# al-mcintyre/mCaller

Measured on NVIDIA B200. Metric: per-read site calls/sec, higher is better.
Workload: dtype f64

## Files before the change

### mcaller_b200/csrc/common.cuh

```cuda
#pragma once
#include <cuda_runtime.h>
#include <stdint.h>
#include <stdio.h>
#include "../../include/mcaller_b200.h"

void mc_set_error(const char *fmt, ...);

#define MC_CUDA_CHECK(expr)                                                                  \
    do {                                                                                     \
        cudaError_t _e = (expr);                                                             \
        if (_e != cudaSuccess) {                                                             \
            mc_set_error("%s:%d %s -> %s", __FILE__, __LINE__, #expr, cudaGetErrorString(_e)); \
            return MC_ECUDA;                                                                 \
        }                                                                                    \
    } while (0)

#define MC_LAUNCH_CHECK() MC_CUDA_CHECK(cudaGetLastError())

#define MC_REQUIRE(cond, msg)                       \
    do {                                            \
        if (!(cond)) {                              \
            mc_set_error("%s: %s", __func__, msg);  \
            return MC_EINVAL;                       \
        }                                           \
    } while (0)

__device__ __forceinline__ uint32_t mc_kmer_bits(const uint32_t *__restrict__ bm, int64_t g, int k) {
    int64_t w = g >> 5;
    int b = (int)(g & 31);
    uint32_t lo = __ldg(bm + w), hi = __ldg(bm + w + 1);
    uint32_t v = __funnelshift_r(lo, hi, b);
    return v & ((1u << k) - 1u);
}

template <int THREADS>
__device__ __forceinline__ int mc_block_exscan(int v, int *s_warp , int &total) {
    const int lane = threadIdx.x & 31, wid = threadIdx.x >> 5;
    int inc = v;
#pragma unroll
    for (int d = 1; d < 32; d <<= 1) {
        int t = __shfl_up_sync(0xffffffffu, inc, d);
        if (lane >= d) inc += t;
    }
    if (lane == 31) s_warp[wid] = inc;
    __syncthreads();
    if (wid == 0) {
        int x = (lane < THREADS / 32) ? s_warp[lane] : 0;
        int xi = x;
#pragma unroll
        for (int d = 1; d < 32; d <<= 1) {
            int t = __shfl_up_sync(0xffffffffu, xi, d);
            if (lane >= d) xi += t;
        }
        if (lane < THREADS / 32) s_warp[lane] = xi - x;
        if (lane == 31) s_warp[THREADS / 32] = xi;
    }
    __syncthreads();
    total = s_warp[THREADS / 32];
    int res = s_warp[wid] + inc - v;
    __syncthreads();
    return res;
}

int mc_exscan_u32(const uint32_t *d_in, uint32_t *d_out, int64_t n_cap, const uint64_t *d_n ,
                  uint64_t *d_total , void *d_ws, cudaStream_t st);
int64_t mc_exscan_ws_bytes(int64_t n);

__device__ __forceinline__ int64_t mc_dev_count(const unsigned long long *d_n, int64_t cap) {
    const unsigned long long v = *d_n;
    return v < (unsigned long long)cap ? (int64_t)v : cap;
}

__device__ __forceinline__ int64_t mc_rec_line(const mc_record &r) { return ((int64_t)r.line_hi << 32) | (int64_t)r.line_lo; }

struct mc_read_key {
    unsigned long long hash;
    uint32_t check;
    uint32_t len;
};
__device__ __forceinline__ mc_read_key mc_read_key_of(const uint8_t *p, int64_t max_len) {
    unsigned long long h = 14695981039346656037ull, h2 = 0x84222325cbf29ce4ull;
    int64_t len = 0;
    for (; len < max_len; ++len) {
        const unsigned c = __ldg(p + len);
        if (c <= 0x20u || c == ':' || c == '_') break;
        h = (h ^ c) * 1099511628211ull;
        h2 = (h2 ^ c) * 1099511628211ull;
    }
    return {h == 0ull ? 1ull : h, (uint32_t)(h2 >> 32), (uint32_t)len};
}

template <class F>
__device__ __forceinline__ double mc_pairwise_block(F f, int64_t i0, int64_t n) {
    if (n < 8) {
        double res = 0.0;
        for (int64_t i = 0; i < n; ++i) res = __dadd_rn(res, f(i0 + i));
        return res;
    }
    double r[8];
#pragma unroll
    for (int j = 0; j < 8; ++j) r[j] = f(i0 + j);
    int64_t i = 8;
    for (; i < n - (n % 8); i += 8) {
#pragma unroll
        for (int j = 0; j < 8; ++j) r[j] = __dadd_rn(r[j], f(i0 + i + j));
    }
    double res = __dadd_rn(__dadd_rn(__dadd_rn(r[0], r[1]), __dadd_rn(r[2], r[3])), __dadd_rn(__dadd_rn(r[4], r[5]), __dadd_rn(r[6], r[7])));
    for (; i < n; ++i) res = __dadd_rn(res, f(i0 + i));
    return res;
}
template <class F>
__device__ double mc_pairwise_sum(F f, int64_t i0, int64_t n) {
    if (n <= 128) return mc_pairwise_block(f, i0, n);
    constexpr int DEPTH = 40;
    int64_t st_i0[DEPTH], st_n[DEPTH];
    double st_left[DEPTH];
    int st_phase[DEPTH];
    int sp = 0;
    st_i0[0] = i0; st_n[0] = n; st_phase[0] = 0; st_left[0] = 0.0;
    double ret = 0.0;
    for (;;) {
        if (st_phase[sp] == 0) {
            if (st_n[sp] <= 128 || sp + 1 >= DEPTH) {
                ret = mc_pairwise_block(f, st_i0[sp], st_n[sp]);
            } else {
                int64_t n2 = st_n[sp] / 2;
                n2 -= n2 % 8;
                st_phase[sp] = 1;
                st_i0[sp + 1] = st_i0[sp]; st_n[sp + 1] = n2; st_phase[sp + 1] = 0;
                ++sp;
                continue;
            }
        }
        for (;;) {
            if (sp == 0) return ret;
            --sp;
            if (st_phase[sp] == 1) {
                int64_t n2 = st_n[sp] / 2;
                n2 -= n2 % 8;
                st_left[sp] = ret;
                st_phase[sp] = 2;
                st_i0[sp + 1] = st_i0[sp] + n2; st_n[sp + 1] = st_n[sp] - n2; st_phase[sp + 1] = 0;
                ++sp;
                break;
            }
            ret = __dadd_rn(st_left[sp], ret);
        }
    }
}

__device__ __forceinline__ double mc_expit(double x) { return x < 0.0 ? exp(x) / (1.0 + exp(x)) : 1.0 / (1.0 + exp(-x)); }

__device__ __forceinline__ double mc_tanh(double x) {
    double y = -2.0 * fabs(x);
    y = fmax(y, -80.0);
    const double n = rint(y * 1.4426950408889634074);
    double r = fma(n, -6.93147180369123816490e-01, y);
    r = fma(n, -1.90821492927058770002e-10, r);
    double p = 1.6059043836821613e-10;
    p = fma(p, r, 2.0876756987868100e-09);
    p = fma(p, r, 2.5052108385441720e-08);
    p = fma(p, r, 2.7557319223985890e-07);
    p = fma(p, r, 2.7557319223985893e-06);
    p = fma(p, r, 2.4801587301587302e-05);
    p = fma(p, r, 1.9841269841269841e-04);
    p = fma(p, r, 1.3888888888888889e-03);
    p = fma(p, r, 8.3333333333333332e-03);
    p = fma(p, r, 4.1666666666666664e-02);
    p = fma(p, r, 1.6666666666666666e-01);
    p = fma(p, r, 0.5);
    p = fma(p, r, 1.0);
    p = fma(p, r, 1.0);
    const double t = p * __longlong_as_double((long long)(1023 + (int)n) << 52);
    const double d = 1.0 + t, u = 1.0 - t;
    double rc = (double)__frcp_rn((float)d);
    double e = fma(-d, rc, 1.0);
    rc = fma(rc, e, rc);
    e = fma(-d, rc, 1.0);
    rc = fma(rc, e, rc);
    double q = u * rc;
    q = fma(fma(-d, q, u), rc, q);
    return copysign(q, x);
}
```

### mcaller_b200/csrc/parse.cuh

```cuda
#pragma once
#include "common.cuh"

__constant__ double c_pow10[23] = {1e0,  1e1,  1e2,  1e3,  1e4,  1e5,  1e6,  1e7,  1e8,  1e9,  1e10, 1e11,
                                   1e12, 1e13, 1e14, 1e15, 1e16, 1e17, 1e18, 1e19, 1e20, 1e21, 1e22};

struct SmemBytes {
    const uint8_t *p;
    __device__ __forceinline__ int operator[](int i) const { return p[i]; }
};
struct GlobalBytes {
    const uint8_t *p;
    int64_t limit;
    __device__ __forceinline__ int operator[](int64_t i) const { return i < limit ? __ldg(p + i) : 0x0a; }
};

template <class B>
__device__ __forceinline__ bool contig_match(const B &t, int q, const mc_refindex &R, int cid) {
    const int o0 = __ldg(R.d_name_off + cid), L = __ldg(R.d_name_off + cid + 1) - o0;
    for (int j = 0; j < L; ++j)
        if (t[q + j] != __ldg(R.d_names + o0 + j)) return false;
    return t[q + L] <= 0x20;
}
template <class B>
__device__ __forceinline__ int contig_cmp(const B &t, int q, const mc_refindex &R, int cid) {
    const int o0 = __ldg(R.d_name_off + cid), L = __ldg(R.d_name_off + cid + 1) - o0;
    for (int j = 0; j < L; ++j) {
        const int a = t[q + j], b = __ldg(R.d_names + o0 + j);
        if (a <= 0x20) return -1;
        if (a != b) return a - b;
    }
    return t[q + L] <= 0x20 ? 0 : 1;
}
template <class B>
__device__ __forceinline__ int contig_lookup(const B &t, int q, const mc_refindex &R, int hint) {
    if (contig_match(t, q, R, hint)) return hint;
    int lo = 0, hi = R.n_contigs - 1;
    while (lo <= hi) {
        const int mid = (lo + hi) >> 1;
        const int c = contig_cmp(t, q, R, mid);
        if (c == 0) return mid;
        if (c < 0) hi = mid - 1; else lo = mid + 1;
    }
    return -1;
}
template <class B>
__device__ __forceinline__ bool parse_uint(const B &t, int q, int &out) {
    int v = 0, nd = 0, c;
    while ((c = t[q]) >= '0' && c <= '9') { v = v * 10 + (c - '0'); ++nd; ++q; if (nd > 9) return false; }
    if (nd == 0 || c > 0x20) return false;
    out = v;
    return true;
}
template <class B>
__device__ __forceinline__ bool parse_int(const B &t, int q, int &out) {
    bool neg = false;
    if (t[q] == '-') { neg = true; ++q; } else if (t[q] == '+') ++q;
    int v;
    if (!parse_uint(t, q, v)) return false;
    out = neg ? -v : v;
    return true;
}
template <class B>
__device__ __forceinline__ bool parse_decimal(const B &t, int q, double &out) {
    bool neg = false;
    int c = t[q];
    if (c == '-') { neg = true; ++q; } else if (c == '+') ++q;
    unsigned long long m = 0;
    int nd = 0, nfrac = 0;
    while ((c = t[q]) >= '0' && c <= '9') { m = m * 10ull + (unsigned)(c - '0'); ++nd; ++q; if (nd > 18) return false; }
    if (c == '.') {
        ++q;
        while ((c = t[q]) >= '0' && c <= '9') { m = m * 10ull + (unsigned)(c - '0'); ++nd; ++nfrac; ++q; if (nd > 18) return false; }
    }
    if (nd == 0 || c > 0x20 || m > (1ull << 53)) return false;
    const double v = __ddiv_rn((double)m, c_pow10[nfrac]);
    out = neg ? -v : v;
    return true;
}
template <class B>
__device__ __forceinline__ bool is_nnnnnn(const B &t, int q) {
    if (t[q] != 'N') return false;
    return t[q + 1] == 'N' && t[q + 2] == 'N' && t[q + 3] == 'N' && t[q + 4] == 'N' && t[q + 5] == 'N' && t[q + 6] <= 0x20;
}


template <class B>
__device__ __forceinline__ bool tokens_equal(const B &t, int64_t a, int64_t b) {
    for (;;) {
        const int ca = t[a++], cb = t[b++];
        const bool ea = ca <= 0x20, eb = cb <= 0x20;
        if (ea || eb) return ea && eb;
        if (ca != cb) return false;
    }
}

template <class B>
__device__ __forceinline__ void parse_values(const B &t, int f2, int f5, int f6, int f9, int f10, int &event_idx, double &diff,
                                             uint32_t &flags) {
    event_idx = 0;
    if (!parse_int(t, f5, event_idx)) flags |= MC_RF_BADIDX;
    double ev = 0.0, md = 0.0;
    if (!parse_decimal(t, f6, ev) || !parse_decimal(t, f10, md)) { flags |= MC_RF_BADNUM; diff = 0.0; }
    else diff = __ddiv_rn(rint(__dmul_rn(__dsub_rn(ev, md), 1e4)), 1e4);
    if (tokens_equal(t, f2, f9)) flags |= MC_RF_EQ;
}

__device__ __forceinline__ uint32_t gt20_msb(uint32_t w) { return (((w & 0x7f7f7f7fu) + 0x5f5f5f5fu) | w) & 0x80808080u; }
__device__ __forceinline__ uint32_t pack16(uint32_t m0, uint32_t m1, uint32_t m2, uint32_t m3) {
    const uint32_t lo = 0x08040201u, hi = 0x80402010u;
    const uint32_t a = __dp4a(m1, hi, __dp4a(m0, lo, 0u)), b = __dp4a(m3, hi, __dp4a(m2, lo, 0u));
    return (a >> 7) | (b << 1);
}
__device__ __forceinline__ int nth_bit(uint32_t m, int j) {
#pragma unroll
    for (int t = 0; t < 6; ++t)
        if (j > t) m &= m - 1u;
    for (int t = 6; t < j; ++t) m &= m - 1u;
    return __ffs(m) - 1;
}
__device__ __forceinline__ uint32_t conv4(uint32_t h) {
    const uint32_t t = ((h * 2561u) >> 8) & 0x00ff00ffu;
    return (t * 6553601u) >> 16;
}

__device__ __forceinline__ unsigned long long nondigit8(unsigned long long v) {
    const unsigned long long x = v ^ 0x3030303030303030ull;
    return (((x & 0x7f7f7f7f7f7f7f7full) + 0x7676767676767676ull) | v) & 0x8080808080808080ull;
}
__device__ __forceinline__ uint32_t digits_value(unsigned long long v, int n) {
    const unsigned long long x = (v ^ 0x3030303030303030ull) << (64 - 8 * n);
    return conv4((uint32_t)x) * 10000u + conv4((uint32_t)(x >> 32));
}
__device__ __forceinline__ bool fast_uint8(unsigned long long v, int &out) {
    const unsigned long long nd = nondigit8(v);
    if (nd == 0ull) return false;
    const int n = (__ffsll((long long)nd) - 1) >> 3;
    if (n == 0 || ((v >> (8 * n)) & 0xFFull) > 0x20ull) return false;
    out = (int)digits_value(v, n);
    return true;
}
__device__ __forceinline__ bool fast_decimal8(unsigned long long v, uint32_t &mant, int &nfrac) {
    const unsigned long long nd = nondigit8(v);
    if (nd == 0ull) return false;
    const int p1 = (__ffsll((long long)nd) - 1) >> 3;
    if (p1 == 0 || p1 > 6 || ((v >> (8 * p1)) & 0xFFull) != 0x2eull) return false;
    const unsigned long long low = (1ull << (8 * p1)) - 1ull;
    const unsigned long long w = (v & low) | ((v >> 8) & ~low);
    const unsigned long long nd2 = ((nd & low) | ((nd >> 8) & ~low)) & 0x0080808080808080ull;
    if (nd2 == 0ull) return false;
    const int p2 = (__ffsll((long long)nd2) - 1) >> 3;
    if (((w >> (8 * p2)) & 0xFFull) > 0x20ull) return false;
    mant = digits_value(w, p2);
    nfrac = p2 - p1;
    return true;
}
__device__ __forceinline__ int fast_tokens_equal8(unsigned long long a, unsigned long long b) {
    auto ws8 = [](unsigned long long v) {
        return ~((((v & 0x7f7f7f7f7f7f7f7full) + 0x5f5f5f5f5f5f5f5full) | v)) & 0x8080808080808080ull;
    };
    const unsigned long long wa = ws8(a), wb = ws8(b);
    if (wa == 0ull || wb == 0ull) return -1;
    const int la = (__ffsll((long long)wa) - 1) >> 3, lb = (__ffsll((long long)wb) - 1) >> 3;
    if (la != lb) return 0;
    return (((a ^ b) & ((1ull << (8 * la)) - 1ull)) == 0ull) ? 1 : 0;
}

__device__ __forceinline__ unsigned long long load8_unaligned(const uint8_t *p) {
    const uintptr_t a = reinterpret_cast<uintptr_t>(p);
    const unsigned long long *q = reinterpret_cast<const unsigned long long *>(a & ~(uintptr_t)7);
    const int sh = 8 * (int)(a & 7);
    const unsigned long long lo = __ldg(q);
    if (sh == 0) return lo;
    const unsigned long long hi = __ldg(q + 1);
    return (lo >> sh) | (hi << (64 - sh));
}
__device__ __forceinline__ bool bytes_differ(const uint8_t *pa, const uint8_t *pb, int L) {
    const uintptr_t ua = reinterpret_cast<uintptr_t>(pa), ub = reinterpret_cast<uintptr_t>(pb);
    const unsigned long long *qa = reinterpret_cast<const unsigned long long *>(ua & ~(uintptr_t)7);
    const unsigned long long *qb = reinterpret_cast<const unsigned long long *>(ub & ~(uintptr_t)7);
    const int sa = 8 * (int)(ua & 7), sb = 8 * (int)(ub & 7);
    unsigned long long a_lo = __ldg(qa), b_lo = __ldg(qb), diff = 0ull;
#pragma unroll 5
    for (int j = 0; j < L; j += 8) {
        const unsigned long long a_hi = __ldg(++qa), b_hi = __ldg(++qb);
        const unsigned long long va = sa ? ((a_lo >> sa) | (a_hi << (64 - sa))) : a_lo;
        const unsigned long long vb = sb ? ((b_lo >> sb) | (b_hi << (64 - sb))) : b_lo;
        unsigned long long d = va ^ vb;
        if (L - j < 8) d &= (1ull << (8 * (L - j))) - 1ull;
        diff |= d;
        a_lo = a_hi;
        b_lo = b_hi;
    }
    return diff != 0ull;
}

__device__ __forceinline__ void mc_finish_values(const uint8_t *lp, int64_t room, int f2, int f5, int f6, int f9, int f10, int &ev_idx,
                                                 double &diff, uint32_t &fl) {
    uint32_t m_ev = 0u, m_md = 0u;
    int n_ev = 0, n_md = 0;
    const int teq = fast_tokens_equal8(load8_unaligned(lp + f2), load8_unaligned(lp + f9));
    if (f10 + 16 < room && teq >= 0 && fast_uint8(load8_unaligned(lp + f5), ev_idx) &&
        fast_decimal8(load8_unaligned(lp + f6), m_ev, n_ev) && fast_decimal8(load8_unaligned(lp + f10), m_md, n_md)) {
        const double ev = __ddiv_rn((double)m_ev, c_pow10[n_ev]), md = __ddiv_rn((double)m_md, c_pow10[n_md]);
        diff = __ddiv_rn(rint(__dmul_rn(__dsub_rn(ev, md), 1e4)), 1e4);
        if (teq) fl |= MC_RF_EQ;
    } else {
        parse_values(GlobalBytes{lp, room}, f2, f5, f6, f9, f10, ev_idx, diff, fl);
    }
}

__device__ __forceinline__ void mc_finish_record(const uint8_t *__restrict__ text, int64_t limit, mc_record &r) {
    const int64_t line = mc_rec_line(r);
    const int64_t a0 = line & ~15ll;
    const int skip = (int)(line - a0);
    int nf = 0, f2 = 0, f3 = 0, name_end = -1, f5 = 0, f6 = 0, f9 = 0, f10 = 0;
    uint32_t prev_nonws = 0u;
    bool done = false;
    constexpr int MAX_STEPS = 256;
    for (int step = 0; step < MAX_STEPS && !done; ++step) {
        const int64_t g = a0 + 16ll * step;
        if (g >= limit) break;
        const uint4 v = __ldg(reinterpret_cast<const uint4 *>(text + g));
        uint32_t nonws = pack16(gt20_msb(v.x), gt20_msb(v.y), gt20_msb(v.z), gt20_msb(v.w));
        if (step == 0) nonws &= 0xFFFFu << skip;
        const int base = 16 * step - skip;
        uint32_t fs = nonws & ~((nonws << 1) | prev_nonws);
        if (name_end < 0 && nf >= 4) {
            const uint32_t z = ~nonws & 0xFFFFu & ((step == 0) ? (0xFFFFu << skip) : 0xFFFFu);
            const uint32_t zz = z & ~((1u << max(f3 - base, 0)) - 1u);
            if (zz) name_end = base + __ffs(zz) - 1;
        }
        while (fs) {
            const int b = __ffs(fs) - 1;
            fs &= fs - 1u;
            const int pos = base + b;
            switch (nf) {
                case 2: f2 = pos; break;
                case 3: f3 = pos; break;
                case 5: f5 = pos; break;
                case 6: f6 = pos; break;
                case 9: f9 = pos; break;
                case 10: f10 = pos; break;
                default: break;
            }
            ++nf;
            if (nf == 4 && name_end < 0) {
                const uint32_t z = ~nonws & 0xFFFFu & ~((1u << b) - 1u);
                if (z) name_end = base + __ffs(z) - 1;
            }
            if (nf == 11) { done = true; break; }
        }
        prev_nonws = (nonws >> 15) & 1u;
    }
    uint32_t fl = r.flags & ~MC_RF_RAW;
    int ev_idx = 0;
    double diff = 0.0;
    if (nf < 11 || name_end < 0 || f3 > 65535 || name_end - f3 > 65535) fl |= MC_RF_BADNUM | MC_RF_BADIDX;
    else mc_finish_values(text + line, limit - line, f2, f5, f6, f9, f10, ev_idx, diff, fl);
    r.name_off = (uint16_t)f3;
    r.name_len = (uint16_t)(name_end < 0 ? 0 : name_end - f3);
    r.event_idx = ev_idx;
    r.diff = diff;
    r.flags = (uint8_t)fl;
}

__device__ __forceinline__ void mc_finish_record_win(const uint8_t *__restrict__ text, int64_t limit, mc_record &r) {
    const uint32_t *rw = reinterpret_cast<const uint32_t *>(&r);
    const uint32_t W0 = rw[3], W1 = rw[4], W2 = rw[5], W3 = (rw[1] >> 16) | (rw[6] << 16);
    const int c0 = __popc(W0), c1 = c0 + __popc(W1), c2 = c1 + __popc(W2), c3 = c2 + __popc(W3);
    const int64_t line = mc_rec_line(r);
    if ((r.pad & 2u) || c3 < 11 || line + 160 >= limit) {
        r.pad = 0;
        mc_finish_record(text, limit, r);
        return;
    }
    uint32_t m = W0;
    int wi = 0;
    auto next = [&]() {
        while (m == 0u && wi < 3) {
            ++wi;
            m = wi == 1 ? W1 : wi == 2 ? W2 : W3;
        }
        const int q = 32 * wi + __ffs(m) - 1;
        m &= m - 1u;
        return q;
    };
    next();
    next();
    const int f2 = next(), f3 = next(), f4 = next(), f5 = next(), f6 = next();
    next();
    next();
    const int f9 = next(), f10 = next();
    const uint8_t *lp = text + line;
    int name_end;
    {
        const unsigned long long t8 = f4 >= 8 ? load8_unaligned(lp + f4 - 8) : 0ull;
        const uint32_t nh = gt20_msb((uint32_t)(t8 >> 32)), nlw = gt20_msb((uint32_t)t8);
        const int tw = nh ? (__clz(nh) >> 3) : nlw ? 4 + (__clz(nlw) >> 3) : 8;
        name_end = f4 - tw;
        if (tw == 8 || name_end <= f3) {
            name_end = f4 - 1;
            while (name_end > f3 && __ldg(lp + name_end - 1) <= 0x20) --name_end;
        }
    }
    uint32_t fl = r.flags & ~MC_RF_RAW;
    int ev_idx = 0;
    double diff = 0.0;
    mc_finish_values(lp, limit - line, f2, f5, f6, f9, f10, ev_idx, diff, fl);
    r.name_off = (uint16_t)f3;
    r.name_len = (uint16_t)(name_end - f3);
    r.event_idx = ev_idx;
    r.diff = diff;
    r.flags = (uint8_t)fl;
    r.pad = 0;
}
```

### mcaller_b200/csrc/records.cu

```cuda
#include "parse.cuh"

namespace {

constexpr int SCAN_THREADS = 256;
constexpr int SCAN_IPT = 8;
constexpr int SCAN_BLOCK = SCAN_THREADS * SCAN_IPT;

__global__ void __launch_bounds__(SCAN_THREADS) k_scan_reduce(const uint32_t *__restrict__ in, int64_t n_cap,
                                                            const unsigned long long *__restrict__ d_n,
                                                            unsigned long long *__restrict__ block_sums) {
    __shared__ int s_warp[SCAN_THREADS / 32 + 1];
    const int64_t n = d_n ? mc_dev_count(d_n, n_cap) : n_cap;
    const int64_t base = (int64_t)blockIdx.x * SCAN_BLOCK;
    unsigned long long acc = 0ull;
#pragma unroll
    for (int j = 0; j < SCAN_IPT; ++j) {
        const int64_t i = base + (int64_t)j * SCAN_THREADS + threadIdx.x;
        if (i < n) acc += in[i];
    }
    for (int d = 16; d > 0; d >>= 1) acc += __shfl_down_sync(0xffffffffu, acc, d);
    __shared__ unsigned long long s_sum[SCAN_THREADS / 32];
    if ((threadIdx.x & 31) == 0) s_sum[threadIdx.x >> 5] = acc;
    __syncthreads();
    if (threadIdx.x == 0) {
        unsigned long long t = 0ull;
        for (int w = 0; w < SCAN_THREADS / 32; ++w) t += s_sum[w];
        block_sums[blockIdx.x] = t;
    }
    (void)s_warp;
}

__global__ void __launch_bounds__(1024) k_scan_sums(unsigned long long *__restrict__ block_sums, int64_t nb,
                                                   unsigned long long *__restrict__ d_total) {
    __shared__ unsigned long long s_w[33];
    __shared__ unsigned long long s_carry;
    if (threadIdx.x == 0) s_carry = 0ull;
    __syncthreads();
    const int lane = threadIdx.x & 31, wid = threadIdx.x >> 5;
    for (int64_t c0 = 0; c0 < nb; c0 += 1024) {
        const int64_t i = c0 + threadIdx.x;
        const unsigned long long v = (i < nb) ? block_sums[i] : 0ull;
        unsigned long long inc = v;
        for (int d = 1; d < 32; d <<= 1) {
            unsigned long long t = __shfl_up_sync(0xffffffffu, inc, d);
            if (lane >= d) inc += t;
        }
        if (lane == 31) s_w[wid] = inc;
        __syncthreads();
        if (wid == 0) {
            unsigned long long x = s_w[lane], xi = x;
            for (int d = 1; d < 32; d <<= 1) {
                unsigned long long t = __shfl_up_sync(0xffffffffu, xi, d);
                if (lane >= d) xi += t;
            }
            s_w[lane] = xi - x;
            if (lane == 31) s_w[32] = xi;
        }
        __syncthreads();
        const unsigned long long carry = s_carry;
        if (i < nb) block_sums[i] = carry + s_w[wid] + inc - v;
        __syncthreads();
        if (threadIdx.x == 0) s_carry = carry + s_w[32];
        __syncthreads();
    }
    if (threadIdx.x == 0 && d_total) *d_total = s_carry;
}

__global__ void __launch_bounds__(SCAN_THREADS) k_scan_down(const uint32_t *__restrict__ in, int64_t n_cap,
                                                          const unsigned long long *__restrict__ d_n,
                                                          const unsigned long long *__restrict__ block_sums,
                                                          uint32_t *__restrict__ out) {
    __shared__ int s_warp[SCAN_THREADS / 32 + 1];
    const int64_t n = d_n ? mc_dev_count(d_n, n_cap) : n_cap;
    if ((int64_t)blockIdx.x * SCAN_BLOCK >= n) return;
    const int64_t base = (int64_t)blockIdx.x * SCAN_BLOCK + (int64_t)threadIdx.x * SCAN_IPT;
    uint32_t v[SCAN_IPT];
    int sum = 0;
#pragma unroll
    for (int j = 0; j < SCAN_IPT; ++j) {
        const int64_t i = base + j;
        v[j] = (i < n) ? in[i] : 0u;
        sum += (int)v[j];
    }
    int total;
    int off = mc_block_exscan<SCAN_THREADS>(sum, s_warp, total);
    uint32_t run = (uint32_t)block_sums[blockIdx.x] + (uint32_t)off;
#pragma unroll
    for (int j = 0; j < SCAN_IPT; ++j) {
        const int64_t i = base + j;
        if (i < n) out[i] = run;
        run += v[j];
    }
}

}

int64_t mc_exscan_ws_bytes(int64_t n) { return ((n + SCAN_BLOCK - 1) / SCAN_BLOCK + 1) * 8 + 256; }

int mc_exscan_u32(const uint32_t *d_in, uint32_t *d_out, int64_t n_cap, const uint64_t *d_n, uint64_t *d_total, void *d_ws,
                  cudaStream_t st) {
    if (n_cap <= 0) {
        if (d_total) MC_CUDA_CHECK(cudaMemsetAsync(d_total, 0, 8, st));
        return MC_OK;
    }
    const int64_t nb = (n_cap + SCAN_BLOCK - 1) / SCAN_BLOCK;
    unsigned long long *sums = reinterpret_cast<unsigned long long *>(d_ws);
    const unsigned long long *dn = reinterpret_cast<const unsigned long long *>(d_n);
    k_scan_reduce<<<(unsigned)nb, SCAN_THREADS, 0, st>>>(d_in, n_cap, dn, sums);
    MC_LAUNCH_CHECK();
    k_scan_sums<<<1, 1024, 0, st>>>(sums, nb, reinterpret_cast<unsigned long long *>(d_total));
    MC_LAUNCH_CHECK();
    k_scan_down<<<(unsigned)nb, SCAN_THREADS, 0, st>>>(d_in, n_cap, dn, sums, d_out);
    MC_LAUNCH_CHECK();
    return MC_OK;
}

extern "C" int64_t mc_windows_workspace_bytes(int64_t rec_cap);
extern "C" int64_t mc_workspace_bytes(int64_t n) {
    if (n < 1) n = 1;
    const int64_t a = ((n * 4 + 255) / 256) * 256;
    const int64_t mine = 2 * a + mc_exscan_ws_bytes(n) + 512;
    const int64_t win = mc_windows_workspace_bytes(n);
    return mine > win ? mine : win;
}
static inline uint32_t *ws_a(void *ws) { return reinterpret_cast<uint32_t *>(ws); }
static inline uint32_t *ws_b(void *ws, int64_t n) { return reinterpret_cast<uint32_t *>(reinterpret_cast<uint8_t *>(ws) + ((n * 4 + 255) / 256) * 256); }
static inline void *ws_s(void *ws, int64_t n) { return reinterpret_cast<uint8_t *>(ws) + 2 * (((n * 4 + 255) / 256) * 256); }

namespace {

__global__ void __launch_bounds__(256) k_run_resolve(uint32_t *__restrict__ run_tab, int64_t n_runs, uint32_t *__restrict__ cnt_clean,
                                                    const unsigned long long *__restrict__ scan_counters, unsigned long long rec_in_cap) {
    const int64_t r = (int64_t)blockIdx.x * blockDim.x + threadIdx.x;
    if (r >= n_runs) return;
    if (scan_counters && (scan_counters[MC_C_OVERFLOW] != 0ull || scan_counters[MC_C_RECORDS] > rec_in_cap)) {
        cnt_clean[r] = 0u;
        return;
    }
    uint32_t count = run_tab[2 * r];
    const uint32_t v = run_tab[2 * r + 1];
    if (v & 1u) {
        int64_t p = r - 1;
        uint32_t st = 0u;
        while (p >= 0 && (st = (run_tab[2 * p + 1] >> 1) & 3u) == 0u) --p;
        if (p >= 0 && st == 1u && count > 0u) {
            run_tab[2 * r + 1] = v | 0x80000000u;
            --count;
        }
    }
    cnt_clean[r] = count;
}

__global__ void __launch_bounds__(256, 4) k_gather_finish(const uint8_t *__restrict__ text, int64_t limit, mc_refindex R,
                                                      const uint32_t *__restrict__ tile_tab, const uint32_t *__restrict__ run_tab,
                                                      const uint32_t *__restrict__ run_dst, int64_t n_tiles, int64_t n_runs, int run_len,
                                                      const mc_record *__restrict__ in, unsigned long long in_cap, mc_record *__restrict__ out,
                                                      unsigned long long out_cap, uint32_t *__restrict__ seg_flags,
                                                      uint32_t *__restrict__ run_first) {
    const int lane = threadIdx.x & 31;
    const int64_t warp0 = ((int64_t)blockIdx.x * blockDim.x + threadIdx.x) >> 5, n_warps = ((int64_t)gridDim.x * blockDim.x) >> 5;
    for (int64_t run = warp0; run < n_runs; run += n_warps) {
    const uint32_t rv = __ldg(run_tab + 2 * run + 1);
    const bool empty_run = __ldg(run_dst + run) == __ldg(run_dst + run + 1);
    if (run_first && lane == 0) run_first[run] = empty_run ? 0xFFFFFFFFu : __ldg(run_dst + run);
    if (__ldg(run_tab + 2 * run) == 0u) continue;
    const bool drop = (rv >> 31) != 0u;
    unsigned long long d_run = __ldg(run_dst + run);
    const int64_t c0 = run * run_len, c1 = min(c0 + (int64_t)run_len, n_tiles);
    long long carry_line = -1;
    uint32_t carry_span = 0u;
    for (int64_t cb = c0; cb < c1; cb += 32) {
        const int64_t c = cb + lane;
        unsigned long long src = 0ull;
        uint32_t cnt = 0u;
        if (c < c1) {
            const uint2 e = __ldg(reinterpret_cast<const uint2 *>(tile_tab) + c);
            src = e.x;
            cnt = e.y & 0xFFFFu;
            if (drop && ((e.y >> 16) & 1u) && cnt > 0u) { src += 1ull; --cnt; }
        }
        uint32_t incl = cnt;
#pragma unroll
        for (int d = 1; d < 32; d <<= 1) {
            const uint32_t t = __shfl_up_sync(0xffffffffu, incl, d);
            if (lane >= d) incl += t;
        }
        const uint32_t excl = incl - cnt, tot = __shfl_sync(0xffffffffu, incl, 31);
        for (uint32_t k0 = 0; k0 < tot; k0 += 32) {
            const uint32_t idx = k0 + lane;
            const bool act = idx < tot;
            int lo = 0, hi = 31;
#pragma unroll
            for (int st = 0; st < 5; ++st) {
                const int mid = (lo + hi + 1) >> 1;
                const uint32_t e_mid = __shfl_sync(0xffffffffu, excl, mid);
                if (e_mid <= idx) lo = mid; else hi = mid - 1;
            }
            const unsigned long long s_own = __shfl_sync(0xffffffffu, src, lo);
            const uint32_t e_own = __shfl_sync(0xffffffffu, excl, lo);
            const unsigned long long slot = s_own + (idx - e_own), dst = d_run + idx;
            const bool ok = act && slot < in_cap && dst < out_cap;
            alignas(16) mc_record r;
            long long line = -1;
            uint32_t span = 0u;
            if (ok) {
                const uint4 *sp = reinterpret_cast<const uint4 *>(in + slot);
                uint4 *dr = reinterpret_cast<uint4 *>(&r);
                dr[0] = __ldg(sp);
                dr[1] = __ldg(sp + 1);
                if (r.flags & MC_RF_RAW) mc_finish_record_win(text, limit, r);
                if (r.flags & MC_RF_CAND) {
                    const int cid = r.contig;
                    if (r.pos < __ldg(R.d_len + cid)) {
                        const int64_t g = __ldg(R.d_base + cid) + r.pos;
                        r.kbits_fwd = (uint8_t)mc_kmer_bits(R.d_site_fwd, g, R.k);
                        r.kbits_rev = (uint8_t)mc_kmer_bits(R.d_site_rev, g, R.k);
                    }
                }
                line = mc_rec_line(r);
                span = (uint32_t)r.name_off | ((uint32_t)r.name_len << 16);
            }
            long long pl = __shfl_up_sync(0xffffffffu, line, 1);
            uint32_t ps = __shfl_up_sync(0xffffffffu, span, 1);
            if (lane == 0) { pl = carry_line; ps = carry_span; }
            if (ok) {
                uint32_t sf = 1u;
                if (pl >= 0) {
                    uint32_t fl = r.flags | MC_RF_SEGKNOWN;
                    sf = 0u;
                    if ((ps >> 16) != r.name_len || bytes_differ(text + pl + (ps & 0xFFFFu), text + line + r.name_off, r.name_len)) {
                        fl |= MC_RF_NEWREAD;
                        sf = 1u;
                    }
                    r.flags = (uint8_t)fl;
                }
                if (seg_flags) seg_flags[dst] = sf;
                uint4 *dp = reinterpret_cast<uint4 *>(out + dst);
                const uint4 *sr = reinterpret_cast<const uint4 *>(&r);
                dp[0] = sr[0];
                dp[1] = sr[1];
            }
            const int last = (int)min(tot - k0, 32u) - 1;
            carry_line = __shfl_sync(0xffffffffu, line, last);
            carry_span = __shfl_sync(0xffffffffu, span, last);
        }
        d_run += tot;
    }
    }
}

__global__ void __launch_bounds__(256) k_seg_flags(const uint8_t *__restrict__ text, mc_record *__restrict__ rec, int64_t n_cap,
                                                  const unsigned long long *__restrict__ d_n, uint32_t *__restrict__ flags,
                                                  const uint32_t *__restrict__ known) {
    const int64_t n = mc_dev_count(d_n, n_cap);
    const int64_t i = (int64_t)blockIdx.x * blockDim.x + threadIdx.x;
    if (i >= n) return;
    if (known) {
        const uint32_t kf = known[i];
        if (kf < 2u) { flags[i] = kf; return; }
    }
    uint32_t f = 1u;
    const mc_record b = rec[i];
    if (b.flags & MC_RF_SEGKNOWN) {
        f = (b.flags & MC_RF_NEWREAD) ? 1u : 0u;
    } else {
        if (i > 0) {
            const mc_record a = rec[i - 1];
            if (a.name_len == b.name_len)
                f = bytes_differ(text + mc_rec_line(a) + a.name_off, text + mc_rec_line(b) + b.name_off, a.name_len) ? 1u : 0u;
        }
        rec[i].flags = (uint8_t)(b.flags | MC_RF_SEGKNOWN | (f ? MC_RF_NEWREAD : 0u));
    }
    flags[i] = f;
}

__global__ void __launch_bounds__(256) k_seg_fix(const uint8_t *__restrict__ text, mc_record *__restrict__ rec, const unsigned long long *__restrict__ d_n,
                                                int64_t n_cap, const uint32_t *__restrict__ run_first, int64_t n_runs, uint32_t *__restrict__ flags) {
    const int64_t run = (int64_t)blockIdx.x * blockDim.x + threadIdx.x;
    if (run >= n_runs) return;
    const uint32_t i = run_first[run];
    if (i == 0xFFFFFFFFu || (int64_t)i >= mc_dev_count(d_n, n_cap)) return;
    uint32_t f = 1u;
    const mc_record b = rec[i];
    if (i > 0u) {
        const mc_record a = rec[i - 1];
        if (a.name_len == b.name_len)
            f = bytes_differ(text + mc_rec_line(a) + a.name_off, text + mc_rec_line(b) + b.name_off, a.name_len) ? 1u : 0u;
    }
    rec[i].flags = (uint8_t)(b.flags | MC_RF_SEGKNOWN | (f ? MC_RF_NEWREAD : 0u));
    flags[i] = f;
}

__global__ void __launch_bounds__(256) k_seg_starts(const uint32_t *__restrict__ flags, const uint32_t *__restrict__ excl, int64_t n_cap,
                                                   const unsigned long long *__restrict__ d_n, uint32_t *__restrict__ seg_start,
                                                   const unsigned long long *__restrict__ d_nseg) {
    const int64_t n = mc_dev_count(d_n, n_cap);
    const int64_t i = (int64_t)blockIdx.x * blockDim.x + threadIdx.x;
    if (i < n && flags[i]) seg_start[excl[i]] = (uint32_t)i;
    if (i == 0) seg_start[*d_nseg] = (uint32_t)n;
}

__global__ void __launch_bounds__(256) k_seg_quality(const uint8_t *__restrict__ text, const mc_record *__restrict__ rec,
                                                    const uint32_t *__restrict__ seg_start, int64_t seg_cap,
                                                    const unsigned long long *__restrict__ d_nseg,
                                                    const mc_qual_entry *__restrict__ table, unsigned long long mask,
                                                    double *__restrict__ seg_qual, unsigned long long *__restrict__ d_err) {
    const int64_t n_seg = mc_dev_count(d_nseg, seg_cap);
    const int64_t s = (int64_t)blockIdx.x * blockDim.x + threadIdx.x;
    if (s >= n_seg) return;
    const mc_record r = rec[seg_start[s]];
    const mc_read_key key = mc_read_key_of(text + mc_rec_line(r) + r.name_off, r.name_len);
    double q = __longlong_as_double(0x7ff8000000000000ll);
    unsigned long long slot = key.hash & mask;
    for (unsigned long long probe = 0; probe <= mask; ++probe) {
        const mc_qual_entry e = table[slot];
        if (e.hash == 0ull) break;
        if (e.hash == key.hash && e.check == key.check && e.len == key.len) { q = e.qual; break; }
        slot = (slot + 1) & mask;
    }
    if (q != q) atomicAdd(d_err, 1ull);
    seg_qual[s] = q;
}

}

extern "C" int mc_order_records(const uint8_t *d_text, int64_t nbytes, const mc_refindex *ref, const uint32_t *d_tile_tab, int64_t n_tiles,
                                uint32_t *d_run_tab, int run_len, const mc_record *d_rec_in, int64_t rec_in_cap,
                                const uint64_t *d_scan_counters, mc_record *d_rec_out, int64_t rec_out_cap, uint64_t *d_n_out,
                                uint32_t *d_seg_flags, uint32_t *d_run_first, void *d_ws, void *stream) {
    MC_REQUIRE(!d_seg_flags == !d_run_first, "d_seg_flags and d_run_first go together");
    MC_REQUIRE(d_text && ref && d_tile_tab && d_run_tab && d_rec_in && d_rec_out && d_n_out && d_ws, "null pointer");
    MC_REQUIRE(run_len >= 1, "run length must be >= 1");
    cudaStream_t st = (cudaStream_t)stream;
    if (n_tiles <= 0) {
        MC_CUDA_CHECK(cudaMemsetAsync(d_n_out, 0, 8, st));
        return MC_OK;
    }
    const int64_t n_runs = (n_tiles + run_len - 1) / run_len;
    uint32_t *cnt = ws_a(d_ws), *dst = ws_b(d_ws, n_runs + 1);
    MC_CUDA_CHECK(cudaMemsetAsync(cnt + n_runs, 0, 4, st));
    k_run_resolve<<<(unsigned)((n_runs + 255) / 256), 256, 0, st>>>(d_run_tab, n_runs, cnt, reinterpret_cast<const unsigned long long *>(d_scan_counters),
                                                                   (unsigned long long)rec_in_cap);
    MC_LAUNCH_CHECK();
    int rc = mc_exscan_u32(cnt, dst, n_runs + 1, nullptr, d_n_out, ws_s(d_ws, n_runs + 1), st);
    if (rc) return rc;
    int64_t gf_blocks = (n_runs * 32 + 255) / 256;
    {
        int dev = 0, sms = 0;
        MC_CUDA_CHECK(cudaGetDevice(&dev));
        MC_CUDA_CHECK(cudaDeviceGetAttribute(&sms, cudaDevAttrMultiProcessorCount, dev));
        const int64_t resident = (int64_t)sms * 4;
        if (gf_blocks > resident) gf_blocks = resident;
    }
    k_gather_finish<<<(unsigned)gf_blocks, 256, 0, st>>>(d_text, nbytes + MC_TEXT_PAD - 64, *ref, d_tile_tab, d_run_tab, dst, n_tiles,
                                                                          n_runs, run_len, d_rec_in, (unsigned long long)rec_in_cap, d_rec_out,
                                                                          (unsigned long long)rec_out_cap, d_seg_flags, d_run_first);
    MC_LAUNCH_CHECK();
    return MC_OK;
}

extern "C" int mc_segment_reads(const uint8_t *d_text, mc_record *d_rec, const uint64_t *d_n_records, int64_t rec_cap,
                                uint32_t *d_seg_flags, const uint32_t *d_run_first, int64_t n_runs, uint32_t *d_seg_start, uint64_t *d_nseg,
                                void *d_ws, void *stream) {
    MC_REQUIRE(d_text && d_rec && d_n_records && d_seg_start && d_nseg && d_ws, "null pointer");
    cudaStream_t st = (cudaStream_t)stream;
    if (rec_cap <= 0) {
        MC_CUDA_CHECK(cudaMemsetAsync(d_nseg, 0, 8, st));
        MC_CUDA_CHECK(cudaMemsetAsync(d_seg_start, 0, 4, st));
        return MC_OK;
    }
    uint32_t *flags = ws_a(d_ws), *excl = ws_b(d_ws, rec_cap);
    const unsigned nb = (unsigned)((rec_cap + 255) / 256);
    const unsigned long long *dn = reinterpret_cast<const unsigned long long *>(d_n_records);
    if (d_seg_flags && d_run_first) {
        flags = d_seg_flags;
        if (n_runs > 0) k_seg_fix<<<(unsigned)((n_runs + 255) / 256), 256, 0, st>>>(d_text, d_rec, dn, rec_cap, d_run_first, n_runs, flags);
    } else {
        k_seg_flags<<<nb, 256, 0, st>>>(d_text, d_rec, rec_cap, dn, flags, nullptr);
    }
    MC_LAUNCH_CHECK();
    int rc = mc_exscan_u32(flags, excl, rec_cap, d_n_records, d_nseg, ws_s(d_ws, rec_cap), st);
    if (rc) return rc;
    k_seg_starts<<<nb, 256, 0, st>>>(flags, excl, rec_cap, dn, d_seg_start, reinterpret_cast<const unsigned long long *>(d_nseg));
    MC_LAUNCH_CHECK();
    return MC_OK;
}

extern "C" int mc_segment_quality(const uint8_t *d_text, const mc_record *d_rec, const uint32_t *d_seg_start, const uint64_t *d_nseg,
                                  int64_t seg_cap, const mc_qual_entry *d_table, int64_t table_size, double *d_seg_qual,
                                  uint64_t *d_err, void *stream) {
    MC_REQUIRE(d_text && d_rec && d_seg_start && d_nseg && d_table && d_seg_qual && d_err, "null pointer");
    MC_REQUIRE(table_size > 0 && (table_size & (table_size - 1)) == 0, "table size must be a power of two");
    if (seg_cap <= 0) return MC_OK;
    k_seg_quality<<<(unsigned)((seg_cap + 255) / 256), 256, 0, (cudaStream_t)stream>>>(
        d_text, d_rec, d_seg_start, seg_cap, reinterpret_cast<const unsigned long long *>(d_nseg), d_table,
        (unsigned long long)(table_size - 1), d_seg_qual, reinterpret_cast<unsigned long long *>(d_err));
    MC_LAUNCH_CHECK();
    return MC_OK;
}
```

Baseline: 49.22 million.

## Fuse segment-start compaction into scan, add L2 prefetches, simplify unaligned compare

The exclusive scan gains a compacting mode that writes segment start indices directly, which removes the separate k_seg_starts kernel and the intermediate excl array. The gather-finish kernel now issues L2 prefetches for upcoming tile and run tables, input tile bytes and record text lines, to hide global-memory latency. bytes_differ is rewritten to align one operand so only one side needs funnel shifts. Together these cut one launch and some memory traffic, at the cost of extra prefetch instructions and more complex alignment logic.

```diff
diff --git a/mcaller_b200/csrc/common.cuh b/mcaller_b200/csrc/common.cuh
--- a/mcaller_b200/csrc/common.cuh
+++ b/mcaller_b200/csrc/common.cuh
@@ -63,13 +63,15 @@
 }
 
 int mc_exscan_u32(const uint32_t *d_in, uint32_t *d_out, int64_t n_cap, const uint64_t *d_n ,
-                  uint64_t *d_total , void *d_ws, cudaStream_t st);
+                  uint64_t *d_total , void *d_ws, cudaStream_t st, bool compact = false);
 int64_t mc_exscan_ws_bytes(int64_t n);
 
 __device__ __forceinline__ int64_t mc_dev_count(const unsigned long long *d_n, int64_t cap) {
     const unsigned long long v = *d_n;
     return v < (unsigned long long)cap ? (int64_t)v : cap;
 }
+
+__device__ __forceinline__ void mc_prefetch_l2(const void *p) { asm volatile("prefetch.global.L2 [%0];" ::"l"(p)); }
 
 __device__ __forceinline__ int64_t mc_rec_line(const mc_record &r) { return ((int64_t)r.line_hi << 32) | (int64_t)r.line_lo; }
 
diff --git a/mcaller_b200/csrc/parse.cuh b/mcaller_b200/csrc/parse.cuh
--- a/mcaller_b200/csrc/parse.cuh
+++ b/mcaller_b200/csrc/parse.cuh
@@ -165,31 +165,30 @@
     return (((a ^ b) & ((1ull << (8 * la)) - 1ull)) == 0ull) ? 1 : 0;
 }
 
+__device__ __forceinline__ unsigned long long funnel8(unsigned long long lo, unsigned long long hi, int sh) {
+    return (lo >> sh) | ((hi << 1) << (63 - sh));
+}
 __device__ __forceinline__ unsigned long long load8_unaligned(const uint8_t *p) {
     const uintptr_t a = reinterpret_cast<uintptr_t>(p);
     const unsigned long long *q = reinterpret_cast<const unsigned long long *>(a & ~(uintptr_t)7);
-    const int sh = 8 * (int)(a & 7);
-    const unsigned long long lo = __ldg(q);
-    if (sh == 0) return lo;
-    const unsigned long long hi = __ldg(q + 1);
-    return (lo >> sh) | (hi << (64 - sh));
+    return funnel8(__ldg(q), __ldg(q + 1), 8 * (int)(a & 7));
 }
 __device__ __forceinline__ bool bytes_differ(const uint8_t *pa, const uint8_t *pb, int L) {
-    const uintptr_t ua = reinterpret_cast<uintptr_t>(pa), ub = reinterpret_cast<uintptr_t>(pb);
-    const unsigned long long *qa = reinterpret_cast<const unsigned long long *>(ua & ~(uintptr_t)7);
-    const unsigned long long *qb = reinterpret_cast<const unsigned long long *>(ub & ~(uintptr_t)7);
-    const int sa = 8 * (int)(ua & 7), sb = 8 * (int)(ub & 7);
-    unsigned long long a_lo = __ldg(qa), b_lo = __ldg(qb), diff = 0ull;
-#pragma unroll 5
-    for (int j = 0; j < L; j += 8) {
-        const unsigned long long a_hi = __ldg(++qa), b_hi = __ldg(++qb);
-        const unsigned long long va = sa ? ((a_lo >> sa) | (a_hi << (64 - sa))) : a_lo;
-        const unsigned long long vb = sb ? ((b_lo >> sb) | (b_hi << (64 - sb))) : b_lo;
-        unsigned long long d = va ^ vb;
-        if (L - j < 8) d &= (1ull << (8 * (L - j))) - 1ull;
-        diff |= d;
+    uintptr_t ua = reinterpret_cast<uintptr_t>(pa), ub = reinterpret_cast<uintptr_t>(pb);
+    if ((ub & 7) > (ua & 7)) { const uintptr_t t = ua; ua = ub; ub = t; }
+    const int sb = (int)(ub & 7), end = sb + L;
+    const uintptr_t ga = ua - (uintptr_t)sb;
+    const int sa = 8 * (int)(ga & 7);
+    const unsigned long long *qa = reinterpret_cast<const unsigned long long *>(ga & ~(uintptr_t)7);
+    const unsigned long long *qb = reinterpret_cast<const unsigned long long *>(ub - (uintptr_t)sb);
+    unsigned long long a_lo = __ldg(qa), mask = ~0ull << (8 * sb), diff = 0ull;
+#pragma unroll 4
+    for (int j = 0; 8 * j < end; ++j) {
+        const unsigned long long a_hi = __ldg(qa + j + 1);
+        if (end - 8 * j < 8) mask &= (1ull << (8 * (end - 8 * j))) - 1ull;
+        diff |= (funnel8(a_lo, a_hi, sa) ^ __ldg(qb + j)) & mask;
+        mask = ~0ull;
         a_lo = a_hi;
-        b_lo = b_hi;
     }
     return diff != 0ull;
 }
diff --git a/mcaller_b200/csrc/records.cu b/mcaller_b200/csrc/records.cu
--- a/mcaller_b200/csrc/records.cu
+++ b/mcaller_b200/csrc/records.cu
@@ -66,12 +66,14 @@
     if (threadIdx.x == 0 && d_total) *d_total = s_carry;
 }
 
+template <bool COMPACT>
 __global__ void __launch_bounds__(SCAN_THREADS) k_scan_down(const uint32_t *__restrict__ in, int64_t n_cap,
                                                           const unsigned long long *__restrict__ d_n,
                                                           const unsigned long long *__restrict__ block_sums,
-                                                          uint32_t *__restrict__ out) {
+                                                          const unsigned long long *__restrict__ d_total, uint32_t *__restrict__ out) {
     __shared__ int s_warp[SCAN_THREADS / 32 + 1];
     const int64_t n = d_n ? mc_dev_count(d_n, n_cap) : n_cap;
+    if (COMPACT && blockIdx.x == 0 && threadIdx.x == 0) out[*d_total] = (uint32_t)n;
     if ((int64_t)blockIdx.x * SCAN_BLOCK >= n) return;
     const int64_t base = (int64_t)blockIdx.x * SCAN_BLOCK + (int64_t)threadIdx.x * SCAN_IPT;
     uint32_t v[SCAN_IPT];
@@ -88,7 +90,11 @@
 #pragma unroll
     for (int j = 0; j < SCAN_IPT; ++j) {
         const int64_t i = base + j;
-        if (i < n) out[i] = run;
+        if (COMPACT) {
+            if (v[j]) out[run] = (uint32_t)i;
+        } else if (i < n) {
+            out[i] = run;
+        }
         run += v[j];
     }
 }
@@ -98,9 +104,11 @@
 int64_t mc_exscan_ws_bytes(int64_t n) { return ((n + SCAN_BLOCK - 1) / SCAN_BLOCK + 1) * 8 + 256; }
 
 int mc_exscan_u32(const uint32_t *d_in, uint32_t *d_out, int64_t n_cap, const uint64_t *d_n, uint64_t *d_total, void *d_ws,
-                  cudaStream_t st) {
+                  cudaStream_t st, bool compact) {
+    MC_REQUIRE(!compact || d_total, "the compacting scan needs d_total");
     if (n_cap <= 0) {
         if (d_total) MC_CUDA_CHECK(cudaMemsetAsync(d_total, 0, 8, st));
+        if (compact) MC_CUDA_CHECK(cudaMemsetAsync(d_out, 0, 4, st));
         return MC_OK;
     }
     const int64_t nb = (n_cap + SCAN_BLOCK - 1) / SCAN_BLOCK;
@@ -110,7 +118,9 @@
     MC_LAUNCH_CHECK();
     k_scan_sums<<<1, 1024, 0, st>>>(sums, nb, reinterpret_cast<unsigned long long *>(d_total));
     MC_LAUNCH_CHECK();
-    k_scan_down<<<(unsigned)nb, SCAN_THREADS, 0, st>>>(d_in, n_cap, dn, sums, d_out);
+    const unsigned long long *tot = reinterpret_cast<const unsigned long long *>(d_total);
+    if (compact) k_scan_down<true><<<(unsigned)nb, SCAN_THREADS, 0, st>>>(d_in, n_cap, dn, sums, tot, d_out);
+    else k_scan_down<false><<<(unsigned)nb, SCAN_THREADS, 0, st>>>(d_in, n_cap, dn, sums, tot, d_out);
     MC_LAUNCH_CHECK();
     return MC_OK;
 }
@@ -160,6 +170,16 @@
     const int lane = threadIdx.x & 31;
     const int64_t warp0 = ((int64_t)blockIdx.x * blockDim.x + threadIdx.x) >> 5, n_warps = ((int64_t)gridDim.x * blockDim.x) >> 5;
     for (int64_t run = warp0; run < n_runs; run += n_warps) {
+    {
+        const int64_t nr = run + n_warps;
+        const int64_t p0 = run * run_len + 4 * lane, p1 = nr * run_len + 4 * lane;
+        if (p0 < n_tiles) mc_prefetch_l2(tile_tab + 2 * p0);
+        if (p1 < n_tiles) mc_prefetch_l2(tile_tab + 2 * p1);
+        if (lane == 0 && nr < n_runs) {
+            mc_prefetch_l2(run_tab + 2 * nr);
+            mc_prefetch_l2(run_dst + nr);
+        }
+    }
     const uint32_t rv = __ldg(run_tab + 2 * run + 1);
     const bool empty_run = __ldg(run_dst + run) == __ldg(run_dst + run + 1);
     if (run_first && lane == 0) run_first[run] = empty_run ? 0xFFFFFFFFu : __ldg(run_dst + run);
@@ -175,6 +195,14 @@
         uint32_t cnt = 0u;
         if (c < c1) {
             const uint2 e = __ldg(reinterpret_cast<const uint2 *>(tile_tab) + c);
+            if (c + 32 < c1) {
+                const uint2 en = __ldg(reinterpret_cast<const uint2 *>(tile_tab) + c + 32);
+                const uint32_t nc = en.y & 0xFFFFu;
+                if (nc > 0u && en.x + nc <= in_cap) {
+                    mc_prefetch_l2(in + en.x);
+                    mc_prefetch_l2(in + en.x + nc - 1);
+                }
+            }
             src = e.x;
             cnt = e.y & 0xFFFFu;
             if (drop && ((e.y >> 16) & 1u) && cnt > 0u) { src += 1ull; --cnt; }
@@ -208,6 +236,11 @@
                 uint4 *dr = reinterpret_cast<uint4 *>(&r);
                 dr[0] = __ldg(sp);
                 dr[1] = __ldg(sp + 1);
+                {
+                    const int64_t ln = mc_rec_line(r) & ~127ll;
+                    mc_prefetch_l2(text + ln);
+                    mc_prefetch_l2(text + ln + 128);
+                }
                 if (r.flags & MC_RF_RAW) mc_finish_record_win(text, limit, r);
                 if (r.flags & MC_RF_CAND) {
                     const int cid = r.contig;
@@ -291,15 +324,6 @@
     flags[i] = f;
 }
 
-__global__ void __launch_bounds__(256) k_seg_starts(const uint32_t *__restrict__ flags, const uint32_t *__restrict__ excl, int64_t n_cap,
-                                                   const unsigned long long *__restrict__ d_n, uint32_t *__restrict__ seg_start,
-                                                   const unsigned long long *__restrict__ d_nseg) {
-    const int64_t n = mc_dev_count(d_n, n_cap);
-    const int64_t i = (int64_t)blockIdx.x * blockDim.x + threadIdx.x;
-    if (i < n && flags[i]) seg_start[excl[i]] = (uint32_t)i;
-    if (i == 0) seg_start[*d_nseg] = (uint32_t)n;
-}
-
 __global__ void __launch_bounds__(256) k_seg_quality(const uint8_t *__restrict__ text, const mc_record *__restrict__ rec,
                                                     const uint32_t *__restrict__ seg_start, int64_t seg_cap,
                                                     const unsigned long long *__restrict__ d_nseg,
@@ -369,7 +393,7 @@
         MC_CUDA_CHECK(cudaMemsetAsync(d_seg_start, 0, 4, st));
         return MC_OK;
     }
-    uint32_t *flags = ws_a(d_ws), *excl = ws_b(d_ws, rec_cap);
+    uint32_t *flags = ws_a(d_ws);
     const unsigned nb = (unsigned)((rec_cap + 255) / 256);
     const unsigned long long *dn = reinterpret_cast<const unsigned long long *>(d_n_records);
     if (d_seg_flags && d_run_first) {
@@ -379,11 +403,7 @@
         k_seg_flags<<<nb, 256, 0, st>>>(d_text, d_rec, rec_cap, dn, flags, nullptr);
     }
     MC_LAUNCH_CHECK();
-    int rc = mc_exscan_u32(flags, excl, rec_cap, d_n_records, d_nseg, ws_s(d_ws, rec_cap), st);
-    if (rc) return rc;
-    k_seg_starts<<<nb, 256, 0, st>>>(flags, excl, rec_cap, dn, d_seg_start, reinterpret_cast<const unsigned long long *>(d_nseg));
-    MC_LAUNCH_CHECK();
-    return MC_OK;
+    return mc_exscan_u32(flags, d_seg_start, rec_cap, d_n_records, d_nseg, ws_s(d_ws, rec_cap), st, true);
 }
 
 extern "C" int mc_segment_quality(const uint8_t *d_text, const mc_record *d_rec, const uint32_t *d_seg_start, const uint64_t *d_nseg,
```

After: 49.77 million, median of 6. 1.1% higher.
